# YIVEK/aom-av1-lavish

Hardware: AMD Instinct MI355X
Metric: superblocks/s (fwd_txfm+quant+SAD RDO inner loop), 1080p cpu-used=6, 1/2/4/8 GPU (higher is better)
Workload: dtype int32; 1 GPU; rdo: 1920x1080 8-bit frame per step; C2 fwd_txfm2d + quantize_fp (qindex 128) of all 14 TX sizes <=32x32 x every valid TX type + C3 DIAMOND full-pel search of every 16x16 block x 7 refs (downsampled SAD, MV_COST_ENTROPY default nmv context, sadperbit 4, errorperbit 31, cost list, step_param 0; candidate rows from the references' tiled copy, rebuilt per step); 510 SB64/frame; parallelism=frame-per-rank x1, legs=C3 on a second stream beside C2 (C3 in at most 384 workgroups)

## Files before the change

### aom-av1-lavish_amd/csrc/mcomp_lj.hip

```cpp
#include <atomic>

#include "mcomp_dev.h"
#include "txq_dev.h"

namespace lavish {
namespace {

constexpr int kLjJobs = 8;
constexpr int kMvDecHalf = 2047;
constexpr int kMvDecN = 2 * kMvDecHalf + 1;

__device__ __forceinline__ uint32_t group_min8(uint32_t v) {
  v = min(v, (uint32_t)__builtin_amdgcn_update_dpp(0, (int)v, 0xB1, 0xF, 0xF, false));
  v = min(v, (uint32_t)__builtin_amdgcn_update_dpp(0, (int)v, 0x4E, 0xF, 0xF, false));
  v = min(v, (uint32_t)__builtin_amdgcn_update_dpp(0, (int)v, 0x141, 0xF, 0xF, false));
  return v;
}

struct LjSrc {
  uint32_t sk[4], fr[2][4];
};

template <bool SKIP>
__device__ __forceinline__ uint32_t lj_sad(const Ctx& c, const LjSrc& s, int l, int r, int cc) {
// ... 3 lines not shown
    uint32_t t[4];
    load_row<4>(c.tiles + tile_off(c, c.oy + r + 2 * l, x), t);
#pragma unroll
    for (int i = 0; i < 4; ++i) acc = sad4(s.sk[i], t[i], acc);
  } else {
#pragma unroll
    for (int k = 0; k < 2; ++k) {
      uint32_t t[4];
      load_row<4>(c.tiles + tile_off(c, c.oy + r + l + 8 * k, x), t);
#pragma unroll
      for (int i = 0; i < 4; ++i) acc = sad4(s.fr[k][i], t[i], acc);
    }
  }
  acc = group_sum8(acc);
  return SKIP ? 2 * acc : acc;
}

__device__ __forceinline__ int lj_var(const Ctx& c, const LjSrc& s, int l, int r, int cc) {
  int sum = 0;
  uint32_t sse = 0;
#pragma unroll
  for (int k = 0; k < 2; ++k) {
    uint32_t t[4];
    load_row<4>(c.ref + (int64_t)(r + l + 8 * k) * c.rs + cc, t);
#pragma unroll
    for (int i = 0; i < 4; ++i) var_acc(s.fr[k][i], t[i], sum, sse);
  }
  const uint32_t ts = group_sum8((uint32_t)sum), tq = group_sum8(sse);
  const uint32_t var = tq - (uint32_t)(((int64_t)(int)ts * (int)ts) / 256);
  return (int)var + mv_cost(c, r, cc);
}

template <bool SKIP, int N>
__device__ __forceinline__ void lj_sads(const Ctx& c, const LjSrc& s, int l,
                                        __amdgpu_buffer_rsrc_t trs, int oob, const int (&r)[N],
                                        const int (&cc)[N], const bool (&v)[N],
                                        uint32_t (&out)[N]) {
  constexpr int RW = SKIP ? 1 : 2;
  u32x4 t[N][RW];
#pragma unroll
  for (int i = 0; i < N; ++i)
#pragma unroll
    for (int k = 0; k < RW; ++k) {
      const int y = c.oy + r[i] + (SKIP ? 2 * l : l + 8 * k);
      t[i][k] = __builtin_amdgcn_raw_buffer_load_b128(
          trs, v[i] ? (int)tile_off(c, y, c.ox + cc[i]) : oob, 0, 0);
    }
#pragma unroll
  for (int i = 0; i < N; ++i) {
    uint32_t acc = 0;
#pragma unroll
    for (int k = 0; k < RW; ++k) {
      const uint32_t* q = SKIP ? s.sk : s.fr[k];
      acc = sad4(q[0], t[i][k].x, acc);
      acc = sad4(q[1], t[i][k].y, acc);
      acc = sad4(q[2], t[i][k].z, acc);
      acc = sad4(q[3], t[i][k].w, acc);
    }
    acc = group_sum8(acc);
    out[i] = SKIP ? 2 * acc : acc;
  }
}

__device__ __forceinline__ uint32_t scatter_sum8(const uint32_t (&p)[8], int l) {
  const bool hi = l & 4, m1 = l & 2, m0 = l & 1;
  uint32_t q[4], r[2];
#pragma unroll
  for (int k = 0; k < 4; ++k) {
    const uint32_t send = hi ? p[k] : p[k + 4];
    const uint32_t keep = hi ? p[k + 4] : p[k];
    q[k] = keep + (uint32_t)__builtin_amdgcn_update_dpp(0, (int)send, 0x141, 0xF, 0xF, false);
  }
#pragma unroll
  for (int k = 0; k < 2; ++k) {
    const uint32_t send = m1 ? q[k] : q[k + 2];
    const uint32_t keep = m1 ? q[k + 2] : q[k];
    r[k] = keep + (uint32_t)__builtin_amdgcn_update_dpp(0, (int)send, 0x4E, 0xF, 0xF, false);
  }
  const uint32_t send = m0 ? r[0] : r[1];
  const uint32_t keep = m0 ? r[1] : r[0];
  return keep + (uint32_t)__builtin_amdgcn_update_dpp(0, (int)send, 0xB1, 0xF, 0xF, false);
}

__device__ __forceinline__ uint32_t lj_step_sad(const LjSrc& s, __amdgpu_buffer_rsrc_t trs,
                                                int oob, const uint32_t (&off)[8],
                                                const bool (&v)[8], int l) {
  u32x4 t[8];
#pragma unroll
  for (int i = 0; i < 8; ++i)
    t[i] = __builtin_amdgcn_raw_buffer_load_b128(trs, v[i] ? (int)off[i] : oob, 0, 0);
  uint32_t p[8];
#pragma unroll
  for (int i = 0; i < 8; ++i) {
    uint32_t acc = sad4(s.sk[0], t[i].x, 0);
    acc = sad4(s.sk[1], t[i].y, acc);
    acc = sad4(s.sk[2], t[i].z, acc);
    p[i] = sad4(s.sk[3], t[i].w, acc);
  }
  return 2 * scatter_sum8(p, l);
}

__device__ __forceinline__ MvRate mvsad_rate_dec(const Ctx& c, const int32_t* dec, int row,
                                                 int col) {
  if (dec == nullptr) return mvsad_rate(c, row, col);
  const int kr = row - c.full_ref_row, kc = col - c.full_ref_col;
  const int joint = (kc != 0) | ((kr != 0) << 1);
  typedef const __attribute__((address_space(1))) int32_t* gi32;
  return MvRate{((gi32)c.mvjcost)[joint], ((gi32)dec)[kr + kMvDecHalf],
                ((gi32)dec)[kc + kMvDecHalf + kMvDecN]};
}

template <bool SKIP>
__device__ void lj_pass(const Ctx& c, const LjSrc& s, int l, __amdgpu_buffer_rsrc_t trs, int oob,
                        const int32_t* dec, bool run, int step_param, bool want_cl,
                        uint32_t* res, int& steps,
                        int& searches, int& br, int& bc, int& sme, int (&cl)[5]) {
  const int srow = min(max(br, c.row_min), c.row_max);
  const int scol = min(max(bc, c.col_min), c.col_max);
  const int sdr = site_dr(l), sdc = site_dc(l);
  uint32_t c0;
  {
    const int r1[1] = {srow}, c1[1] = {scol};
    const bool v1[1] = {true};
    uint32_t o1[1];
    lj_sads<SKIP, 1>(c, s, l, trs, oob, r1, c1, v1, o1);
    c0 = o1[0] + mvsad_finish(c, mvsad_rate_dec(c, dec, srow, scol), srow, scol);
  }
  const int further = kMaxSteps - 1 - step_param;
  bool active = run;
  bool first = true;
  int n = 0, row = srow, col = scol, stp = kMaxSteps - step_param - 1, center = 0, nres = 0;
  bool offc = false;
  uint32_t best = c0;
  while (__builtin_amdgcn_ballot_w64(active) != 0) {
    const int rad = 1 << stp;
    const int rl = row + sdr * rad, cl_ = col + sdc * rad;
    const bool vl = cl_ >= c.col_min && cl_ <= c.col_max && rl >= c.row_min && rl <= c.row_max;
    MvRate mr = {0, 0, 0};
    if (vl && active) mr = mvsad_rate_dec(c, dec, rl, cl_);
    uint32_t mine = 0;
    constexpr int NS = SKIP ? 8 : 4;
    if constexpr (SKIP) {
      const bool up = row - rad >= c.row_min, dn = row + rad <= c.row_max;
      const bool lf = col - rad >= c.col_min, rt = col + rad <= c.col_max;
      const int y0 = c.oy + row + 2 * l, x0 = c.ox + col;
      uint32_t off[8];
      bool vv[8];
      if (stp > 0) {
        const int yb = (y0 & 1) * c.fsz + ((y0 >> 1) << 5), d16 = rad << 4;
        const int f32 = c.fh << 5;
        auto xo = [&](int x) { return __mul24(x >> 4, f32) + (x & 15); };
        const int xm = xo(x0 - rad), xc = xo(x0), xp = xo(x0 + rad);
#pragma unroll
        for (int t = 0; t < 8; ++t) {
          const int dr = site_dr(t), dc = site_dc(t);
          off[t] = (uint32_t)((dr < 0 ? yb - d16 : dr > 0 ? yb + d16 : yb) +
                              (dc < 0 ? xm : dc > 0 ? xp : xc));
        }
      } else {
#pragma unroll
        for (int t = 0; t < 8; ++t) off[t] = tile_off(c, y0 + site_dr(t), x0 + site_dc(t));
      }
#pragma unroll
      for (int t = 0; t < 8; ++t) {
        const int dr = site_dr(t), dc = site_dc(t);
        vv[t] = active && (dr < 0 ? up : dr > 0 ? dn : true) && (dc < 0 ? lf : dc > 0 ? rt : true);
      }
      if (active) mine = lj_step_sad(s, trs, oob, off, vv, l);
    } else
    if (active)
#pragma unroll
    for (int h = 0; h < 8 / NS; ++h) {
      int rr[NS], cc[NS];
      bool vv[NS];
      uint32_t sd[NS];
#pragma unroll
      for (int i = 0; i < NS; ++i) {
        const int t = h * NS + i;
        rr[i] = row + site_dr(t) * rad;
        cc[i] = col + site_dc(t) * rad;
        vv[i] = active && cc[i] >= c.col_min && cc[i] <= c.col_max && rr[i] >= c.row_min &&
                rr[i] <= c.row_max;
      }
      lj_sads<SKIP, NS>(c, s, l, trs, oob, rr, cc, vv, sd);
#pragma unroll
      for (int i = 0; i < NS; ++i) mine = l == h * NS + i ? sd[i] : mine;
    }
    const uint32_t key =
        (((mine + mvsad_finish(c, mr, rl, cl_)) << 3) | (uint32_t)l) | (vl ? 0u : ~0u);
    const uint32_t kmin = group_min8(key);
    if (active) {
      ++steps;
      if (kmin < (best << 3)) {
        best = kmin >> 3;
        const int i = (int)(kmin & 7);
        row += site_dr(i) * rad;
        col += site_dc(i) * rad;
        offc = true;
      }
      if (!offc) ++center;
      if (--stp < 0) {
        if (l == 0) res[nres] = ((uint32_t)(uint16_t)row << 16) | (uint16_t)col;
        ++nres;
        ++searches;
        if (first) n = center;
        else if (center) n += center;
        first = false;
        if (n < further) {
          ++n;
          row = srow;
          col = scol;
          best = c0;
          stp = kMaxSteps - (step_param + n) - 1;
          center = 0;
          offc = false;
        } else {
          active = false;
          stp = 0;
        }
      }
    }
  }
  wave_sync();
  if (!run) return;
  for (int i = 0; i < nres; ++i) {
    const uint32_t p = res[i];
    const int r = (int16_t)(p >> 16), cc = (int16_t)(p & 0xFFFF);
    const int v = lj_var(c, s, l, r, cc);
    if (i == 0 || v < sme) {
      sme = v;
      br = r;
      bc = cc;
    }
  }
  if (want_cl) {
    int rr[5], cc[5];
    bool vv[5];
    uint32_t sd[5];
    MvRate m[5];
#pragma unroll
    for (int t = 0; t < 5; ++t) {
      rr[t] = br + (t == 2 ? 1 : t == 4 ? -1 : 0);
      cc[t] = bc + (t == 1 ? -1 : t == 3 ? 1 : 0);
      vv[t] = t == 0 ||
              (cc[t] >= c.col_min && cc[t] <= c.col_max && rr[t] >= c.row_min && rr[t] <= c.row_max);
      m[t] = mvsad_rate_dec(c, dec, vv[t] ? rr[t] : br, vv[t] ? cc[t] : bc);
    }
    lj_sads<SKIP, 5>(c, s, l, trs, oob, rr, cc, vv, sd);
#pragma unroll
    for (int t = 0; t < 5; ++t)
      cl[t] = vv[t] ? (int)(sd[t] + mvsad_finish(c, m[t], rr[t], cc[t])) : INT_MAX;
  }
}

__device__ __forceinline__ void lj_jobs(
    const uint8_t* __restrict__ src, int ss, const uint8_t* __restrict__ ref, int rs,
    const LavishRefTiles& tiles, const Job* __restrict__ jobs, int njobs, int step_param,
    const LavishMvCostParams& cost, const int32_t* dec, int skip,
    LavishDiamondResult* __restrict__ out, int32_t* __restrict__ cost_lists, int j0,
    uint32_t* res);

template <int WPG>
__device__ __forceinline__ void lj_group(
    const uint8_t* __restrict__ src, int ss, const uint8_t* __restrict__ ref, int rs,
    const LavishRefTiles& tiles, const Job* __restrict__ jobs, int njobs, int step_param,
    const LavishMvCostParams& cost, const int32_t* dec, int skip,
    LavishDiamondResult* __restrict__ out, int32_t* __restrict__ cost_lists, int vwg, int nvwg) {
  __shared__ uint32_t res_s[WPG][kLjJobs][kMaxSteps];
  const int wg = (vwg & 7) * (nvwg >> 3) + (vwg >> 3);
  const int lane = threadIdx.x & 63;
  const int wave = WPG == 1 ? 0 : threadIdx.x >> 6;
  const int j0 = (wg * WPG + wave) * kLjJobs;
  if (j0 >= njobs) return;
  lj_jobs(src, ss, ref, rs, tiles, jobs, njobs, step_param, cost, dec, skip, out, cost_lists, j0,
          res_s[wave][lane >> 3]);
}

__device__ __forceinline__ void lj_jobs(
    const uint8_t* __restrict__ src, int ss, const uint8_t* __restrict__ ref, int rs,
    const LavishRefTiles& tiles, const Job* __restrict__ jobs, int njobs, int step_param,
    const LavishMvCostParams& cost, const int32_t* dec, int skip,
    LavishDiamondResult* __restrict__ out, int32_t* __restrict__ cost_lists, int j0,
    uint32_t* res) {
  const int lane = threadIdx.x & 63;
  const int jg = lane >> 3, l = lane & 7;
  const int j = min(j0 + jg, njobs - 1);
  const bool mine_job = j0 + jg < njobs;
  const Job jb = jobs[j];
  Ctx c;
  c.src = src + jb.src_off;
  c.ref = ref + jb.ref_off;
  c.ss = ss;
  c.rs = rs;
  c.col_min = jb.col_min;
  c.col_max = jb.col_max;
  c.row_min = jb.row_min;
  c.row_max = jb.row_max;
  c.ref_mv_row = jb.ref_mv_row;
  c.ref_mv_col = jb.ref_mv_col;
  c.full_ref_row = rawpel(jb.ref_mv_row);
  c.full_ref_col = rawpel(jb.ref_mv_col);
  c.cost_type = cost.mv_cost_type;
  c.sad_lambda = sad_lambda(cost.mv_cost_type);
  c.sse_lambda = sse_lambda(cost.mv_cost_type);
  c.sad_per_bit = cost.sad_per_bit;
  c.error_per_bit = cost.error_per_bit;
  const bool ent = cost.mv_cost_type == 0;
  c.mvjcost = ent ? cost.mvjcost : kZeroRate;
  c.mvcost0 = ent ? cost.mvcost[0] : kZeroRate;
  c.mvcost1 = ent ? cost.mvcost[1] : kZeroRate;
  c.tiles = tiles.data;
  c.fh = tiles.field_rows;
  c.fsz = (int)tiles.field_bytes;
  c.oy = (int)(jb.ref_off / rs);
  c.ox = (int)(jb.ref_off - (int64_t)c.oy * rs);
  const int oob = (int)(2 * tiles.field_bytes);
  const __amdgpu_buffer_rsrc_t trs =
      __builtin_amdgcn_make_buffer_rsrc((void*)tiles.data, 0, oob, 0x00020000);
  LjSrc s;
  load_row<4>(c.src + (int64_t)(2 * l) * ss, s.sk);
  load_row<4>(c.src + (int64_t)l * ss, s.fr[0]);
  load_row<4>(c.src + (int64_t)(l + 8) * ss, s.fr[1]);
  const bool want_cl = cost_lists != nullptr;
  int cl[5] = {INT_MAX, INT_MAX, INT_MAX, INT_MAX, INT_MAX};
  int steps = 0, searches = 0, sme = 0;
  int br = jb.start_row, bc = jb.start_col;
  bool full = true;
  if (skip) {
    lj_pass<true>(c, s, l, trs, oob, dec, true, step_param, want_cl, res, steps, searches, br, bc,
                  sme, cl);
    uint32_t all = 0;
#pragma unroll
    for (int k = 0; k < 2; ++k) {
      uint32_t t[4];
      load_row<4>(c.ref + (int64_t)(br + l + 8 * k) * rs + bc, t);
#pragma unroll
      for (int i = 0; i < 4; ++i) all = sad4(s.fr[k][i], t[i], all);
    }
    const int sad = (int)group_sum8(all);
    const int ssad = (int)(2 * group_sum8((l & 1) ? 0u : all));
    full = sad > 16 && abs(ssad - sad) * 10 >= max(sad, 1) * 9;
    if (full) {
      br = jb.start_row;
      bc = jb.start_col;
    }
  }
  if (__builtin_amdgcn_ballot_w64(full) != 0)
    lj_pass<false>(c, s, l, trs, oob, dec, full, step_param, want_cl, res, steps, searches, br, bc,
                   sme, cl);
  if (!mine_job) return;
  if (l == 0) {
    LavishDiamondResult r;
    r.best_row = (int16_t)br;
    r.best_col = (int16_t)bc;
    r.bestsme = sme;
    r.steps = steps;
    r.searches = searches;
    out[j] = r;
  }
  if (want_cl && l < 5) {
    const int v = l == 0 ? cl[0] : l == 1 ? cl[1] : l == 2 ? cl[2] : l == 3 ? cl[3] : cl[4];
    cost_lists[5 * (int64_t)j + l] = v;
  }
}

#ifndef LAVISH_LJ_WAVES
#define LAVISH_LJ_WAVES 4
#endif
template <int WPG>
__global__ __launch_bounds__(64 * WPG, LAVISH_LJ_WAVES) void diamond_lj_kernel(
    const uint8_t* __restrict__ src, int ss, const uint8_t* __restrict__ ref, int rs,
    LavishRefTiles tiles, const Job* __restrict__ jobs, int njobs, int step_param,
    LavishMvCostParams cost, const int32_t* dec, int skip, LavishDiamondResult* __restrict__ out,
    int32_t* __restrict__ cost_lists, int nvwg) {
  for (int v = blockIdx.x; v < nvwg; v += gridDim.x)
    lj_group<WPG>(src, ss, ref, rs, tiles, jobs, njobs, step_param, cost, dec, skip, out,
                  cost_lists, v, nvwg);
}

constexpr int kLjQueueStride = 16;

template <int WPG>
__global__ __launch_bounds__(64 * WPG, LAVISH_LJ_WAVES) void diamond_lj_dyn_kernel(
    const uint8_t* __restrict__ src, int ss, const uint8_t* __restrict__ ref, int rs,
    LavishRefTiles tiles, const Job* __restrict__ jobs, int njobs, int step_param,
    LavishMvCostParams cost, const int32_t* dec, int skip, LavishDiamondResult* __restrict__ out,
    int32_t* __restrict__ cost_lists, int* __restrict__ queue) {
  __shared__ uint32_t res_s[WPG][kLjJobs][kMaxSteps];
  const int units = (njobs + kLjJobs - 1) / kLjJobs;
  const int x = blockIdx.x & 7;
  const int u0 = units * x / 8, u1 = units * (x + 1) / 8;
  const int lane = threadIdx.x & 63;
  const int wave = WPG == 1 ? 0 : threadIdx.x >> 6;
  uint32_t* res = res_s[wave][lane >> 3];
  int* q = queue + x * kLjQueueStride;
  for (;;) {
    int t = 0;
    if (lane == 0) t = __hip_atomic_fetch_add(q, 1, __ATOMIC_RELAXED, __HIP_MEMORY_SCOPE_AGENT);
    t = __builtin_amdgcn_readfirstlane(t);
    if (u0 + t >= u1) break;
    lj_jobs(src, ss, ref, rs, tiles, jobs, njobs, step_param, cost, dec, skip, out, cost_lists,
            (u0 + t) * kLjJobs, res);
  }
}

__global__ void lj_queue_zero(int* __restrict__ queue) {
  if (threadIdx.x < 8 * kLjQueueStride) queue[threadIdx.x] = 0;
}

struct LjLaunch {
  const uint8_t* src;
  int ss;
  const uint8_t* ref;
  int rs;
  LavishRefTiles tiles;
  const Job* jobs;
  int njobs, step_param;
  LavishMvCostParams cost;
  const int32_t* dec;
  int skip;
  LavishDiamondResult* out;
  int32_t* cost_lists;
  int nvwg;
  int units;
  int every;
};

__global__ __launch_bounds__(256, 4) void txq_search_kernel(TxqDispatch d, TxqArgs a0, TxqArgs a1,
                                                            TxqArgs a2, TxqArgs a3, TxqArgs a4,
                                                            TxqArgs a5, TxqArgs a6, TxqArgs a7,
                                                            TxqArgs a8, LjLaunch c) {
  __shared__ __attribute__((aligned(16))) char lds[class_lds(0)];
  const int u = blockIdx.x >> 3, x = blockIdx.x & 7;
  const int k = u / c.every;
  if (u - k * c.every == 0 && k < c.units) {
    lj_group<4>(c.src, c.ss, c.ref, c.rs, c.tiles, c.jobs, c.njobs, c.step_param, c.cost, c.dec,
                c.skip, c.out, c.cost_lists, k * 8 + x, c.nvwg);
    return;
  }
  const int before = min((u + c.every - 1) / c.every, c.units);
  txq_multi_body<0>(d, a0, a1, a2, a3, a4, a5, a6, a7, a8, (u - before) * 8 + x, lds);
}

__global__ __launch_bounds__(256) void mvcost_dec_kernel(const int32_t* __restrict__ mvcost0,
                                                         const int32_t* __restrict__ mvcost1,
                                                         int32_t* __restrict__ dec,
                                                         int* __restrict__ queue) {
  const int i = blockIdx.x * 256 + threadIdx.x;
  if (queue != nullptr && i < 8 * kLjQueueStride) queue[i] = 0;
  if (i >= 2 * kMvDecN) return;
  const int k = (i % kMvDecN) - kMvDecHalf;
  dec[i] = (i < kMvDecN ? mvcost0 : mvcost1)[8 * k];
}

thread_local StreamScratch t_mvdec;

static std::atomic<int> g_lj_cap{0};
static int lj_grid_cap() { return g_lj_cap.load(std::memory_order_relaxed); }
static std::atomic<int> g_lj_queue{1};

constexpr int kTilesK = 8, kTilesF = 32, kTilesC = kTilesK + 1;
__global__ __launch_bounds__(256) void ref_tiles_kernel(const uint8_t* __restrict__ ref,
                                                        int stride, int rows, int nstrips,
                                                        int fh, uint8_t* __restrict__ out,
                                                        int ktiles, int ftiles) {
  __shared__ u32x4 seg[kTilesF][kTilesC];
  const int t = threadIdx.x;
  int b = blockIdx.x;
  const int kt = b % ktiles;
  b /= ktiles;
  const int ft = b % ftiles;
  const int f = b / ftiles;
  const int k0 = kt * kTilesK, fy0 = ft * kTilesF;
  for (int idx = t; idx < kTilesF * kTilesC; idx += 256) {
    const int i = idx / kTilesC, m = idx - i * kTilesC;
    const int y = 2 * (fy0 + i) + f, x = 16 * (k0 + m);
    u32x4 v = {0u, 0u, 0u, 0u};
    if (y < rows && x < stride) {
      const uint8_t* p = ref + (int64_t)y * stride + x;
      if (x + 16 <= stride) {
        const u32x4u w = *(const __attribute__((address_space(1))) u32x4u*)p;
        v = u32x4{w.x, w.y, w.z, w.w};
      } else {
        uint32_t q[4] = {0u, 0u, 0u, 0u};
        for (int j = 0; j < 16 && x + j < stride; ++j) q[j >> 2] |= (uint32_t)p[j] << (8 * (j & 3));
        v = u32x4{q[0], q[1], q[2], q[3]};
      }
    }
    seg[i][m] = v;
  }
  __syncthreads();
  for (int q = t; q < kTilesK * kTilesF * 2; q += 256) {
    const int kk = q >> 6, i = (q >> 1) & (kTilesF - 1), h = q & 1;
    const int k = k0 + kk, fy = fy0 + i;
    if (k < nstrips && fy < fh)
      *(u32x4*)(out + ((((int64_t)f * nstrips + k) * fh + fy) << 5) + 16 * h) = seg[i][kk + h];
  }
}

}

void launch_lj(const uint8_t* src, int ss, const uint8_t* ref, int rs, const LavishRefTiles& t,
               const LavishDiamondJob* jobs, int njobs, int step_param,
               const LavishMvCostParams& cost, int skip, LavishDiamondResult* out,
               int32_t* cost_lists, hipStream_t s) {
  const int waves = (njobs + kLjJobs - 1) / kLjJobs;
  constexpr int wpg = 4;
  const int nwg = (((waves + wpg - 1) / wpg) + 7) & ~7;
  const int cap = lj_grid_cap();
  const int grid = cap > 0 && cap < nwg ? cap : nwg;
  const bool dyn = grid < nwg && g_lj_queue.load(std::memory_order_relaxed);
  constexpr size_t kDecBytes = 2 * kMvDecN * sizeof(int32_t);
  const size_t qbytes = dyn ? 8 * kLjQueueStride * sizeof(int) : 0;
  int32_t* dec = nullptr;
  int* queue = nullptr;
  char* scr = nullptr;
  if (cost.mv_cost_type == 0 || dyn) {
    scr = (char*)t_mvdec.acquire(kDecBytes + qbytes, s);
    if (dyn) queue = (int*)(scr + kDecBytes);
  }
  if (cost.mv_cost_type == 0) {
    dec = (int32_t*)scr;
    hipLaunchKernelGGL(mvcost_dec_kernel, dim3((2 * kMvDecN + 255) / 256), dim3(256), 0,
                       s, cost.mvcost[0], cost.mvcost[1], dec, queue);
  } else if (dyn) {
    hipLaunchKernelGGL(lj_queue_zero, dim3(1), dim3(8 * kLjQueueStride), 0, s, queue);
  }
  if (dyn)
    hipLaunchKernelGGL(diamond_lj_dyn_kernel<wpg>, dim3(grid), dim3(64 * wpg), 0, s, src,
                       ss, ref, rs, t, (const Job*)jobs, njobs, step_param, cost,
                       (const int32_t*)dec, skip, out, cost_lists, queue);
  else
    hipLaunchKernelGGL(diamond_lj_kernel<wpg>, dim3(grid), dim3(64 * wpg), 0, s, src, ss,
                       ref, rs, t, (const Job*)jobs, njobs, step_param, cost,
                       (const int32_t*)dec, skip, out, cost_lists, nwg);
  if (scr) t_mvdec.release(s);
}

}

using namespace lavish;

extern "C" int lavish_set_search_schedule(int queued) {
  if (queued != 0 && queued != 1) return -1;
  lavish::g_lj_queue.store(queued, std::memory_order_relaxed);
  return 0;
}

extern "C" int lavish_set_search_workgroup_cap(int workgroups) {
  if (workgroups < 0) return -1;
  lavish::g_lj_cap.store((workgroups + 7) & ~7, std::memory_order_relaxed);
  return 0;
}

static int64_t tiles_nstrips(int stride) { return (stride + 15) / 16; }

extern "C" int64_t lavish_ref_tiles_bytes(int stride, int rows) {
  if (stride <= 0 || rows <= 0) return -1;
  return 2 * tiles_nstrips(stride) * ((rows + 1) / 2) * 32;
}

extern "C" int lavish_ref_tiles_build(const uint8_t* ref, int stride, int rows, uint8_t* data,
                                      LavishRefTiles* tiles, void* stream) {
  const int64_t bytes = lavish_ref_tiles_bytes(stride, rows);
  if (ref == nullptr || data == nullptr || tiles == nullptr || bytes <= 0) return -1;
  if (bytes >= ((int64_t)1 << 31)) return -1;
  const int nstrips = (int)tiles_nstrips(stride), fh = (rows + 1) / 2;
  tiles->data = data;
  tiles->field_bytes = (int64_t)nstrips * fh * 32;
  tiles->field_rows = fh;
  tiles->stride = stride;
  const int ktiles = (nstrips + kTilesK - 1) / kTilesK, ftiles = (fh + kTilesF - 1) / kTilesF;
  hipLaunchKernelGGL(ref_tiles_kernel, dim3((unsigned)(2 * ktiles * ftiles)), dim3(256), 0,
                     (hipStream_t)stream, ref, stride, rows, nstrips, fh, data, ktiles, ftiles);
  LAVISH_CHECK(hipGetLastError());
  return 0;
}

extern "C" int lavish_txq_frame_search(
    const int16_t* residual, int stride, int width, int height, uint32_t size_mask,
    const uint32_t* type_masks, int bit_depth, int quant_kind, const LavishQuantParams* qp,
    int32_t* const* qcoeff, int32_t* const* dqcoeff, uint16_t* const* eob, const uint8_t* src,
    int src_stride, const uint8_t* ref, int ref_stride, const LavishRefTiles* tiles,
    const LavishDiamondJob* jobs, int njobs, int step_param, const LavishMvCostParams* cost,
    int use_downsampled_sad, LavishDiamondResult* out, int32_t* cost_lists, int every,
    void* stream) {
  const hipStream_t s = (hipStream_t)stream;
  if (every < 1) return -6;
  if (tiles == nullptr || tiles->data == nullptr || tiles->stride != ref_stride) return -5;
  if (step_param < 0 || step_param >= kMaxSteps) return -1;
  if (!mv_cost_ok(cost)) return -2;
  uint32_t cls0 = 0;
  for (int t = 0; t < 19; ++t)
    if (((size_mask >> t) & 1) && tx_w(t) <= 32 && tx_h(t) <= 32 && !txq_class(t)) cls0 |= 1u << t;
  int rc = 0;
  if (size_mask & ~cls0) {
    rc = txq_frame(residual, stride, width, height, size_mask & ~cls0, type_masks, bit_depth,
                   quant_kind, qp, qcoeff, dqcoeff, eob, s);
    if (rc) return rc;
  }
  TxqMulti m;
  int g = 0;
  rc = txq_frame_plan(residual, stride, width, height, cls0, type_masks, bit_depth, quant_kind, qp,
                      qcoeff, dqcoeff, eob, 0, m, g);
  if (rc) return rc;
  LjLaunch c{};
  c.src = src;
  c.ss = src_stride;
  c.ref = ref;
  c.rs = ref_stride;
  c.tiles = *tiles;
  c.jobs = (const Job*)jobs;
  c.njobs = njobs > 0 ? njobs : 0;
  c.step_param = step_param;
  c.cost = *cost;
  c.skip = use_downsampled_sad;
  c.out = out;
  c.cost_lists = cost_lists;
  const int waves = (c.njobs + kLjJobs - 1) / kLjJobs;
  c.nvwg = (((waves + 3) / 4) + 7) & ~7;
  c.units = c.nvwg / 8;
  if (c.units > 0 && cost->mv_cost_type == 0) {
    c.dec = (const int32_t*)t_mvdec.acquire(2 * kMvDecN * sizeof(int32_t), s);
    hipLaunchKernelGGL(mvcost_dec_kernel, dim3((2 * kMvDecN + 255) / 256), dim3(256), 0, s,
                       cost->mvcost[0], cost->mvcost[1], (int32_t*)c.dec, (int*)nullptr);
  }
  const int u2 = g / 8, ut = u2 + c.units;
// ... 9 lines not shown
```

### aom-av1-lavish_amd/lavish_dsp/motion.py

```python
import ctypes

import numpy as np

from . import _lib, _stream_ptr

JOB_DTYPE = np.dtype([("src_off", "<i8"), ("ref_off", "<i8"), ("start_row", "<i2"),
                      ("start_col", "<i2"), ("ref_mv_row", "<i2"), ("ref_mv_col", "<i2"),
                      ("col_min", "<i2"), ("col_max", "<i2"), ("row_min", "<i2"),
                      ("row_max", "<i2")], align=True)
RESULT_DTYPE = np.dtype([("best_row", "<i2"), ("best_col", "<i2"), ("bestsme", "<i4"),
                         ("steps", "<i4"), ("searches", "<i4")], align=True)
assert JOB_DTYPE.itemsize == 32 and RESULT_DTYPE.itemsize == 16

MV_COST_ENTROPY, MV_COST_L1_LOWRES, MV_COST_L1_MIDRES, MV_COST_L1_HDRES, MV_COST_NONE = range(5)
SEARCH_METHODS = {"diamond": 0, "nstep": 1, "nstep_8pt": 2, "hex": 4, "bigdia": 5, "square": 6,
                  "fast_hex": 7, "fast_diamond": 8, "fast_bigdia": 9, "vfast_diamond": 10}
MV_MAX = (1 << 14) - 1
MI_SIZE = 4
AOM_INTERP_EXTEND = 4
MAX_FULL_PEL_VAL = (1 << 10) - 1
MV_LOW, MV_UPP = -(1 << 14), 1 << 14

_vp, _i32 = ctypes.c_void_p, ctypes.c_int32
_lib.lavish_diamond_search_batch.argtypes = [_vp, _i32, _vp, _i32, _i32, _i32, _vp, _i32, _i32,
# ... 30 lines not shown
_lib.lavish_full_pixel_search_batch_tiled.restype = _i32


class MeshParams(ctypes.Structure):
    _fields_ = [("run_mesh_search", ctypes.c_int32), ("force_mesh_thresh", ctypes.c_int32),
                ("prune_mesh_search", ctypes.c_int32),
                ("mesh_search_mv_diff_threshold", ctypes.c_int32),
                ("fine_search_interval", ctypes.c_int32), ("is_intra_mode", ctypes.c_int32),
                ("range", ctypes.c_int32 * 4), ("interval", ctypes.c_int32 * 4)]

    @classmethod
    def make(cls, patterns, run_mesh_search=0, force_mesh_thresh=0x7FFFFFFF,
             prune_mesh_search=0, mesh_search_mv_diff_threshold=4, fine_search_interval=0,
             is_intra_mode=0):
        m = cls(run_mesh_search, force_mesh_thresh, prune_mesh_search,
                mesh_search_mv_diff_threshold, fine_search_interval, is_intra_mode)
        for i, (r, iv) in enumerate(patterns):
            m.range[i], m.interval[i] = r, iv
        return m


_lib.lavish_full_pixel_search_batch_mesh.argtypes = [
    _vp, _i32, _vp, _i32, ctypes.POINTER(RefTilesDesc), _i32, _i32, _vp, _i32, _i32, _i32,
    ctypes.POINTER(MvCostParams), _i32, ctypes.POINTER(MeshParams), _vp, _vp, _vp]
_lib.lavish_full_pixel_search_batch_mesh.restype = _i32
if hasattr(_lib, "lavish_set_search_workgroup_cap"):
    _lib.lavish_set_search_workgroup_cap.argtypes = [_i32]
    _lib.lavish_set_search_workgroup_cap.restype = _i32
if hasattr(_lib, "lavish_set_search_schedule"):
    _lib.lavish_set_search_schedule.argtypes = [_i32]
    _lib.lavish_set_search_schedule.restype = _i32


class RefTiles:

    def __init__(self, ref, stride=None):
        import torch
        assert ref.dtype == torch.uint8 and ref.is_contiguous()
        self.ref = ref
        self.stride = int(stride if stride is not None else ref.shape[-1])
        self.rows = ref.numel() // self.stride
        n = _lib.lavish_ref_tiles_bytes(self.stride, self.rows)
        if n <= 0:
            raise ValueError("lavish_ref_tiles_bytes rejected (%d, %d)" % (self.stride, self.rows))
        self.data = torch.empty(n, dtype=torch.uint8, device=ref.device)
        self.desc = RefTilesDesc()

    def build(self, stream=None):
        rc = _lib.lavish_ref_tiles_build(_vp(self.ref.data_ptr()), self.stride, self.rows,
                                         _vp(self.data.data_ptr()), ctypes.byref(self.desc),
                                         _stream_ptr(stream))
        if rc != 0:
            raise ValueError("lavish_ref_tiles_build rejected its arguments (rc=%d)" % rc)
        return self


class MvCosts:

    def __init__(self, mvjcost, mvcost, device="cuda"):
        import torch
        mvcost = np.ascontiguousarray(mvcost, np.int32)
        if mvcost.shape != (2, 2 * MV_MAX + 1) or np.shape(mvjcost) != (4,):
            raise ValueError("mvjcost[4] and mvcost[2][%d] expected" % (2 * MV_MAX + 1))
        self.mvjcost = torch.from_numpy(np.ascontiguousarray(mvjcost, np.int32)).to(device)
        self.mvcost = torch.from_numpy(mvcost).to(device)

    def cost_params(self, sad_per_bit, error_per_bit, mv_cost_type=MV_COST_ENTROPY):
        c = MvCostParams(mv_cost_type, sad_per_bit, error_per_bit, 0)
        c.mvjcost = self.mvjcost.data_ptr()
        row = self.mvcost.stride(0) * 4
        c.mvcost[0] = self.mvcost.data_ptr() + 4 * MV_MAX
        c.mvcost[1] = self.mvcost.data_ptr() + row + 4 * MV_MAX
        c._owner = self
        return c


def set_search_workgroup_cap(workgroups):
    rc = _lib.lavish_set_search_workgroup_cap(int(workgroups))
    if rc:
        raise ValueError("lavish_set_search_workgroup_cap(%r): %d" % (workgroups, rc))


def set_search_schedule(queued):
    rc = _lib.lavish_set_search_schedule(1 if queued else 0)
    if rc:
        raise ValueError("lavish_set_search_schedule(%r): %d" % (queued, rc))


def default_mv_cost_tables(allow_hp=False):
    import os
    d = np.load(os.path.join(os.path.dirname(os.path.abspath(__file__)), "data",
                             "nmv_cost_default.npz"))
    t = "hp" if allow_hp else "lp"
    return d["mvjcost_" + t], d["mvcost_" + t]


def sad_per_bit(qindex, bit_depth=8):
    from . import build_quant_params
    q = int(build_quant_params(bit_depth, qindex).dequant[1]) / 4.0
    if bit_depth == 10:
        q /= 4.0
    elif bit_depth == 12:
        q /= 16.0
    return int(0.0418 * q + 2.4107)


def error_per_bit(rdmult):
    return max(rdmult >> 6, 1)


def l1_cost_params(mv_cost_type=MV_COST_L1_HDRES):
    return MvCostParams(mv_cost_type, 0, 0, 0)


def block_mv_limits(mi_rows, mi_cols, mi_row, mi_col, mi_height, mi_width, border):
    e2 = 2 * AOM_INTERP_EXTEND
    row_min = max(-(mi_row * MI_SIZE + border - e2), -((mi_row + mi_height) * MI_SIZE + e2))
    row_max = min((mi_rows - mi_row - mi_height) * MI_SIZE + border - e2,
                  (mi_rows - mi_row) * MI_SIZE + e2)
    col_min = max(-(mi_col * MI_SIZE + border - e2), -((mi_col + mi_width) * MI_SIZE + e2))
    col_max = min((mi_cols - mi_col - mi_width) * MI_SIZE + border - e2,
                  (mi_cols - mi_col) * MI_SIZE + e2)
    return col_min, col_max, row_min, row_max


def subpel_limits(lim, ref_mv=(0, 0)):
    col_min, col_max, row_min, row_max = lim
    max_mv = MAX_FULL_PEL_VAL * 8
    r, c = ref_mv
    minc = max(col_min * 8, c - max_mv)
    maxc = min(col_max * 8, c + max_mv)
    minr = max(row_min * 8, r - max_mv)
    maxr = min(row_max * 8, r + max_mv)
    maxc, maxr = max(minc, maxc), max(minr, maxr)
    return (max(MV_LOW + 1, minc), min(MV_UPP - 1, maxc), max(MV_LOW + 1, minr),
            min(MV_UPP - 1, maxr))


def mv_limits(mi_rows, mi_cols, mi_row, mi_col, mi_height, mi_width, border, ref_mv=(0, 0)):
    col_min, col_max, row_min, row_max = block_mv_limits(mi_rows, mi_cols, mi_row, mi_col,
                                                         mi_height, mi_width, border)
    r, c = ref_mv
    cmin = max(((c + 7) >> 3) - MAX_FULL_PEL_VAL, (MV_LOW >> 3) + 1)
    rmin = max(((r + 7) >> 3) - MAX_FULL_PEL_VAL, (MV_LOW >> 3) + 1)
    cmax = min((c >> 3) + MAX_FULL_PEL_VAL, (MV_UPP >> 3) - 1)
    rmax = min((r >> 3) + MAX_FULL_PEL_VAL, (MV_UPP >> 3) - 1)
    col_min, row_min = max(col_min, cmin), max(row_min, rmin)
    col_max, row_max = min(col_max, cmax), min(row_max, rmax)
    return col_min, max(col_min, col_max), row_min, max(row_min, row_max)


def frame_jobs(width, height, stride, border, plane_bytes, bw, bh, nrefs, ref_mv=(0, 0),
               start_mv=(0, 0), mv_border=None):
    mi_rows = ((height + 7) & ~7) // MI_SIZE
    mi_cols = ((width + 7) & ~7) // MI_SIZE
    nbx, nby = width // bw, height // bh
    n = nbx * nby
    one = np.zeros(n, JOB_DTYPE)
    ys = np.repeat(np.arange(nby) * bh, nbx)
    xs = np.tile(np.arange(nbx) * bw, nby)
    one["src_off"] = (ys + border) * stride + xs + border
    mb = border if mv_border is None else mv_border
    lim = np.array([mv_limits(mi_rows, mi_cols, y // MI_SIZE, x // MI_SIZE, bh // MI_SIZE,
                              bw // MI_SIZE, mb, ref_mv) for y, x in zip(ys, xs)])
    one["col_min"], one["col_max"], one["row_min"], one["row_max"] = lim.T
    one["start_row"], one["start_col"] = start_mv
    one["ref_mv_row"], one["ref_mv_col"] = ref_mv
# ... 218 lines not shown
```

Measured before the change: 776,700 SB64/s.

## Add refill walk kernel that recycles 8-lane groups across diamond searches

Adds schedule mode 2, which splits the skip-mode diamond search into a persistent walk kernel and a separate finish kernel. In the walk kernel each wave keeps a small shared-memory pool of jobs and hands a new job to any 8-lane group whose walk has ended. This removes idle lanes caused by searches of uneven length. Walk results go to a scratch record per job, and the finish kernel reads them back to do variance selection and cost lists. The mode only runs when schedule 2 is selected, and it adds an extra launch plus global traffic for the records.

Measured after the change: 768,900 SB64/s. -1.0%, worse.

```diff
diff --git a/aom-av1-lavish_amd/csrc/mcomp_lj.hip b/aom-av1-lavish_amd/csrc/mcomp_lj.hip
--- a/aom-av1-lavish_amd/csrc/mcomp_lj.hip
+++ b/aom-av1-lavish_amd/csrc/mcomp_lj.hip
@@ -109,6 +109,7 @@
   return keep + (uint32_t)__builtin_amdgcn_update_dpp(0, (int)send, 0xB1, 0xF, 0xF, false);
 }
 
+template <bool ISSUE_ALL = false>
 __device__ __forceinline__ uint32_t lj_step_sad(const LjSrc& s, __amdgpu_buffer_rsrc_t trs,
                                                 int oob, const uint32_t (&off)[8],
                                                 const bool (&v)[8], int l) {
@@ -116,6 +117,7 @@
 #pragma unroll
   for (int i = 0; i < 8; ++i)
     t[i] = __builtin_amdgcn_raw_buffer_load_b128(trs, v[i] ? (int)off[i] : oob, 0, 0);
+  if constexpr (ISSUE_ALL) __builtin_amdgcn_sched_barrier(0);
   uint32_t p[8];
 #pragma unroll
   for (int i = 0; i < 8; ++i) {
@@ -137,11 +139,87 @@
                 ((gi32)dec)[kc + kMvDecHalf + kMvDecN]};
 }
 
+__device__ __forceinline__ void lj_skip_sites(const Ctx& c, int row, int col, int stp, int l,
+                                              bool active, uint32_t (&off)[8], bool (&vv)[8]) {
+  const int rad = 1 << stp;
+  const bool up = row - rad >= c.row_min, dn = row + rad <= c.row_max;
+  const bool lf = col - rad >= c.col_min, rt = col + rad <= c.col_max;
+  const int y0 = c.oy + row + 2 * l, x0 = c.ox + col;
+  if (stp > 0) {
+    const int yb = (y0 & 1) * c.fsz + ((y0 >> 1) << 5), d16 = rad << 4;
+    const int f32 = c.fh << 5;
+    auto xo = [&](int x) { return __mul24(x >> 4, f32) + (x & 15); };
+    const int xm = xo(x0 - rad), xc = xo(x0), xp = xo(x0 + rad);
+#pragma unroll
+    for (int t = 0; t < 8; ++t) {
+      const int dr = site_dr(t), dc = site_dc(t);
+      off[t] = (uint32_t)((dr < 0 ? yb - d16 : dr > 0 ? yb + d16 : yb) +
+                          (dc < 0 ? xm : dc > 0 ? xp : xc));
+    }
+  } else {
+#pragma unroll
+    for (int t = 0; t < 8; ++t) off[t] = tile_off(c, y0 + site_dr(t), x0 + site_dc(t));
+  }
+#pragma unroll
+  for (int t = 0; t < 8; ++t) {
+    const int dr = site_dr(t), dc = site_dc(t);
+    vv[t] = active && (dr < 0 ? up : dr > 0 ? dn : true) && (dc < 0 ? lf : dc > 0 ? rt : true);
+  }
+}
+
+struct LjWalk {
+  int row, col, stp, center, n, nres;
+  bool first, offc;
+  uint32_t best;
+};
+
+__device__ __forceinline__ void lj_walk_begin(LjWalk& w, int srow, int scol, uint32_t c0,
+                                              int step_param) {
+  w.row = srow;
+  w.col = scol;
+  w.best = c0;
+  w.stp = kMaxSteps - step_param - 1;
+  w.center = w.n = w.nres = 0;
+  w.first = true;
+  w.offc = false;
+}
+
+template <class Put>
+__device__ __forceinline__ bool lj_advance(LjWalk& w, uint32_t kmin, int srow, int scol,
+                                           uint32_t c0, int step_param, Put&& put) {
+  const int rad = 1 << w.stp;
+  if (kmin < (w.best << 3)) {
+    w.best = kmin >> 3;
+    const int i = (int)(kmin & 7);
+    w.row += site_dr(i) * rad;
+    w.col += site_dc(i) * rad;
+    w.offc = true;
+  }
+  if (!w.offc) ++w.center;
+  if (--w.stp >= 0) return false;
+  put(w.nres, ((uint32_t)(uint16_t)w.row << 16) | (uint16_t)w.col);
+  ++w.nres;
+  if (w.first) w.n = w.center;
+  else if (w.center) w.n += w.center;
+  w.first = false;
+  if (w.n < kMaxSteps - 1 - step_param) {
+    ++w.n;
+    w.row = srow;
+    w.col = scol;
+    w.best = c0;
+    w.stp = kMaxSteps - (step_param + w.n) - 1;
+    w.center = 0;
+    w.offc = false;
+    return false;
+  }
+  w.stp = 0;
+  return true;
+}
+
 template <bool SKIP>
-__device__ void lj_pass(const Ctx& c, const LjSrc& s, int l, __amdgpu_buffer_rsrc_t trs, int oob,
-                        const int32_t* dec, bool run, int step_param, bool want_cl,
-                        uint32_t* res, int& steps,
-                        int& searches, int& br, int& bc, int& sme, int (&cl)[5]) {
+__device__ void lj_walk(const Ctx& c, const LjSrc& s, int l, __amdgpu_buffer_rsrc_t trs, int oob,
+                        const int32_t* dec, bool run, int step_param, int br, int bc,
+                        uint32_t* res, int& nres, int& steps, int& searches) {
   const int srow = min(max(br, c.row_min), c.row_max);
   const int scol = min(max(bc, c.col_min), c.col_max);
   const int sdr = site_dr(l), sdc = site_dc(l);
@@ -153,46 +231,21 @@
     lj_sads<SKIP, 1>(c, s, l, trs, oob, r1, c1, v1, o1);
     c0 = o1[0] + mvsad_finish(c, mvsad_rate_dec(c, dec, srow, scol), srow, scol);
   }
-  const int further = kMaxSteps - 1 - step_param;
   bool active = run;
-  bool first = true;
-  int n = 0, row = srow, col = scol, stp = kMaxSteps - step_param - 1, center = 0, nres = 0;
-  bool offc = false;
-  uint32_t best = c0;
+  LjWalk w;
+  lj_walk_begin(w, srow, scol, c0, step_param);
   while (__builtin_amdgcn_ballot_w64(active) != 0) {
-    const int rad = 1 << stp;
-    const int rl = row + sdr * rad, cl_ = col + sdc * rad;
+    const int rad = 1 << w.stp;
+    const int rl = w.row + sdr * rad, cl_ = w.col + sdc * rad;
     const bool vl = cl_ >= c.col_min && cl_ <= c.col_max && rl >= c.row_min && rl <= c.row_max;
     MvRate mr = {0, 0, 0};
     if (vl && active) mr = mvsad_rate_dec(c, dec, rl, cl_);
     uint32_t mine = 0;
     constexpr int NS = SKIP ? 8 : 4;
     if constexpr (SKIP) {
-      const bool up = row - rad >= c.row_min, dn = row + rad <= c.row_max;
-      const bool lf = col - rad >= c.col_min, rt = col + rad <= c.col_max;
-      const int y0 = c.oy + row + 2 * l, x0 = c.ox + col;
       uint32_t off[8];
       bool vv[8];
-      if (stp > 0) {
-        const int yb = (y0 & 1) * c.fsz + ((y0 >> 1) << 5), d16 = rad << 4;
-        const int f32 = c.fh << 5;
-        auto xo = [&](int x) { return __mul24(x >> 4, f32) + (x & 15); };
-        const int xm = xo(x0 - rad), xc = xo(x0), xp = xo(x0 + rad);
-#pragma unroll
-        for (int t = 0; t < 8; ++t) {
-          const int dr = site_dr(t), dc = site_dc(t);
-          off[t] = (uint32_t)((dr < 0 ? yb - d16 : dr > 0 ? yb + d16 : yb) +
-                              (dc < 0 ? xm : dc > 0 ? xp : xc));
-        }
-      } else {
-#pragma unroll
-        for (int t = 0; t < 8; ++t) off[t] = tile_off(c, y0 + site_dr(t), x0 + site_dc(t));
-      }
-#pragma unroll
-      for (int t = 0; t < 8; ++t) {
-        const int dr = site_dr(t), dc = site_dc(t);
-        vv[t] = active && (dr < 0 ? up : dr > 0 ? dn : true) && (dc < 0 ? lf : dc > 0 ? rt : true);
-      }
+      lj_skip_sites(c, w.row, w.col, w.stp, l, active, off, vv);
       if (active) mine = lj_step_sad(s, trs, oob, off, vv, l);
     } else
     if (active)
@@ -204,8 +257,8 @@
 #pragma unroll
       for (int i = 0; i < NS; ++i) {
         const int t = h * NS + i;
-        rr[i] = row + site_dr(t) * rad;
-        cc[i] = col + site_dc(t) * rad;
+        rr[i] = w.row + site_dr(t) * rad;
+        cc[i] = w.col + site_dc(t) * rad;
         vv[i] = active && cc[i] >= c.col_min && cc[i] <= c.col_max && rr[i] >= c.row_min &&
                 rr[i] <= c.row_max;
       }
@@ -218,38 +271,21 @@
     const uint32_t kmin = group_min8(key);
     if (active) {
       ++steps;
-      if (kmin < (best << 3)) {
-        best = kmin >> 3;
-        const int i = (int)(kmin & 7);
-        row += site_dr(i) * rad;
-        col += site_dc(i) * rad;
-        offc = true;
-      }
-      if (!offc) ++center;
-      if (--stp < 0) {
-        if (l == 0) res[nres] = ((uint32_t)(uint16_t)row << 16) | (uint16_t)col;
-        ++nres;
-        ++searches;
-        if (first) n = center;
-        else if (center) n += center;
-        first = false;
-        if (n < further) {
-          ++n;
-          row = srow;
-          col = scol;
-          best = c0;
-          stp = kMaxSteps - (step_param + n) - 1;
-          center = 0;
-          offc = false;
-        } else {
-          active = false;
-          stp = 0;
-        }
-      }
-    }
-  }
+      if (lj_advance(w, kmin, srow, scol, c0, step_param, [&](int i, uint32_t p) {
+            if (l == 0) res[i] = p;
+            ++searches;
+          }))
+        active = false;
+    }
+  }
+  nres = w.nres;
   wave_sync();
-  if (!run) return;
+}
+
+template <bool SKIP>
+__device__ void lj_finish(const Ctx& c, const LjSrc& s, int l, __amdgpu_buffer_rsrc_t trs,
+                          int oob, const int32_t* dec, bool want_cl, const uint32_t* res,
+                          int nres, int& br, int& bc, int& sme, int (&cl)[5]) {
   for (int i = 0; i < nres; ++i) {
     const uint32_t p = res[i];
     const int r = (int16_t)(p >> 16), cc = (int16_t)(p & 0xFFFF);
@@ -280,35 +316,51 @@
   }
 }
 
+template <bool SKIP>
+__device__ void lj_pass(const Ctx& c, const LjSrc& s, int l, __amdgpu_buffer_rsrc_t trs, int oob,
+                        const int32_t* dec, bool run, int step_param, bool want_cl,
+                        uint32_t* res, int& steps,
+                        int& searches, int& br, int& bc, int& sme, int (&cl)[5]) {
+  int nres = 0;
+  lj_walk<SKIP>(c, s, l, trs, oob, dec, run, step_param, br, bc, res, nres, steps, searches);
+  if (!run) return;
+  lj_finish<SKIP>(c, s, l, trs, oob, dec, want_cl, res, nres, br, bc, sme, cl);
+}
+
+constexpr int kLjRecWords = 16, kLjRecRes = 4;
+
+template <bool WALKED = false>
 __device__ __forceinline__ void lj_jobs(
     const uint8_t* __restrict__ src, int ss, const uint8_t* __restrict__ ref, int rs,
     const LavishRefTiles& tiles, const Job* __restrict__ jobs, int njobs, int step_param,
     const LavishMvCostParams& cost, const int32_t* dec, int skip,
     LavishDiamondResult* __restrict__ out, int32_t* __restrict__ cost_lists, int j0,
-    uint32_t* res);
-
-template <int WPG>
+    uint32_t* res, const uint32_t* __restrict__ walk = nullptr);
+
+template <int WPG, bool WALKED = false>
 __device__ __forceinline__ void lj_group(
     const uint8_t* __restrict__ src, int ss, const uint8_t* __restrict__ ref, int rs,
     const LavishRefTiles& tiles, const Job* __restrict__ jobs, int njobs, int step_param,
     const LavishMvCostParams& cost, const int32_t* dec, int skip,
-    LavishDiamondResult* __restrict__ out, int32_t* __restrict__ cost_lists, int vwg, int nvwg) {
+    LavishDiamondResult* __restrict__ out, int32_t* __restrict__ cost_lists, int vwg, int nvwg,
+    const uint32_t* __restrict__ walk = nullptr) {
   __shared__ uint32_t res_s[WPG][kLjJobs][kMaxSteps];
   const int wg = (vwg & 7) * (nvwg >> 3) + (vwg >> 3);
   const int lane = threadIdx.x & 63;
   const int wave = WPG == 1 ? 0 : threadIdx.x >> 6;
   const int j0 = (wg * WPG + wave) * kLjJobs;
   if (j0 >= njobs) return;
-  lj_jobs(src, ss, ref, rs, tiles, jobs, njobs, step_param, cost, dec, skip, out, cost_lists, j0,
-          res_s[wave][lane >> 3]);
-}
-
+  lj_jobs<WALKED>(src, ss, ref, rs, tiles, jobs, njobs, step_param, cost, dec, skip, out,
+                  cost_lists, j0, res_s[wave][lane >> 3], walk);
+}
+
+template <bool WALKED>
 __device__ __forceinline__ void lj_jobs(
     const uint8_t* __restrict__ src, int ss, const uint8_t* __restrict__ ref, int rs,
     const LavishRefTiles& tiles, const Job* __restrict__ jobs, int njobs, int step_param,
     const LavishMvCostParams& cost, const int32_t* dec, int skip,
     LavishDiamondResult* __restrict__ out, int32_t* __restrict__ cost_lists, int j0,
-    uint32_t* res) {
+    uint32_t* res, const uint32_t* __restrict__ walk) {
   const int lane = threadIdx.x & 63;
   const int jg = lane >> 3, l = lane & 7;
   const int j = min(j0 + jg, njobs - 1);
@@ -354,8 +406,20 @@
   int br = jb.start_row, bc = jb.start_col;
   bool full = true;
   if (skip) {
-    lj_pass<true>(c, s, l, trs, oob, dec, true, step_param, want_cl, res, steps, searches, br, bc,
-                  sme, cl);
+    if constexpr (WALKED) {
+      typedef const __attribute__((address_space(1))) uint32_t* gu32;
+      const gu32 rec = (gu32)(walk + (int64_t)j * kLjRecWords);
+      const int nres = (int)rec[0];
+      steps = (int)rec[1];
+      searches = (int)rec[2];
+      if (l < nres) res[l] = rec[kLjRecRes + l];
+      if (l + 8 < nres) res[l + 8] = rec[kLjRecRes + 8 + l];
+      wave_sync();
+      lj_finish<true>(c, s, l, trs, oob, dec, want_cl, res, nres, br, bc, sme, cl);
+    } else {
+      lj_pass<true>(c, s, l, trs, oob, dec, true, step_param, want_cl, res, steps, searches, br,
+                    bc, sme, cl);
+    }
     uint32_t all = 0;
 #pragma unroll
     for (int k = 0; k < 2; ++k) {
@@ -433,6 +497,193 @@
 
 __global__ void lj_queue_zero(int* __restrict__ queue) {
   if (threadIdx.x < 8 * kLjQueueStride) queue[threadIdx.x] = 0;
+}
+
+constexpr int kLjPool = 16;
+constexpr int kLjPoolLow = 4;
+
+struct LjPoolRec {
+  Job jb;
+  int oy, ox, j, pad;
+};
+
+template <int WPG>
+__global__ __launch_bounds__(64 * WPG, LAVISH_LJ_WAVES) void diamond_lj_walk_kernel(
+    const uint8_t* __restrict__ src, int ss, int rs, LavishRefTiles tiles,
+    const Job* __restrict__ jobs, int njobs, int step_param, LavishMvCostParams cost,
+    const int32_t* dec, uint32_t* __restrict__ walk, int* __restrict__ queue) {
+  __shared__ LjPoolRec pool_s[WPG][kLjPool];
+  const int units = (njobs + kLjJobs - 1) / kLjJobs;
+  const int x = blockIdx.x & 7;
+  const int u0 = units * x / 8, u1 = units * (x + 1) / 8;
+  const int lane = threadIdx.x & 63;
+  const int wave = WPG == 1 ? 0 : threadIdx.x >> 6;
+  const int l = lane & 7;
+  const int sdr = site_dr(l), sdc = site_dc(l);
+  int* q = queue + x * kLjQueueStride;
+  Ctx c = {};
+  c.ss = ss;
+  c.rs = rs;
+  c.cost_type = cost.mv_cost_type;
+  c.sad_lambda = sad_lambda(cost.mv_cost_type);
+  c.sse_lambda = sse_lambda(cost.mv_cost_type);
+  c.sad_per_bit = cost.sad_per_bit;
+  c.error_per_bit = cost.error_per_bit;
+  const bool ent = cost.mv_cost_type == 0;
+  c.mvjcost = ent ? cost.mvjcost : kZeroRate;
+  c.mvcost0 = ent ? cost.mvcost[0] : kZeroRate;
+  c.mvcost1 = ent ? cost.mvcost[1] : kZeroRate;
+  c.tiles = tiles.data;
+  c.fh = tiles.field_rows;
+  c.fsz = (int)tiles.field_bytes;
+  const int oob = (int)(2 * tiles.field_bytes);
+  const __amdgpu_buffer_rsrc_t trs =
+      __builtin_amdgcn_make_buffer_rsrc((void*)tiles.data, 0, oob, 0x00020000);
+  int head = 0, cnt = 0, stage = 0, rec_n = 0, rec_j0 = 0, tq = 0;
+  bool dry = false;
+  u32x2 rj[4] = {};
+  LjSrc s = {};
+  LjWalk w = {};
+  bool walking = false;
+  int srow = 0, scol = 0, jid = 0, steps = 0;
+  uint32_t c0 = 0;
+  for (;;) {
+    head = __builtin_amdgcn_readfirstlane(head);
+    cnt = __builtin_amdgcn_readfirstlane(cnt);
+    stage = __builtin_amdgcn_readfirstlane(stage);
+    rec_n = __builtin_amdgcn_readfirstlane(rec_n);
+    rec_j0 = __builtin_amdgcn_readfirstlane(rec_j0);
+    dry = __builtin_amdgcn_readfirstlane((int)dry) != 0;
+    if (stage == 2) {
+      if (lane < rec_n) {
+        LjPoolRec r;
+        __builtin_memcpy(&r.jb, rj, sizeof(Job));
+        r.oy = (int)(r.jb.ref_off / rs);
+        r.ox = (int)(r.jb.ref_off - (int64_t)r.oy * rs);
+        r.j = rec_j0 + lane;
+        r.pad = 0;
+        pool_s[wave][(head + cnt + lane) & (kLjPool - 1)] = r;
+      }
+      cnt += rec_n;
+      stage = 0;
+    } else if (stage == 1) {
+      const int t = __builtin_amdgcn_readfirstlane(tq);
+      if (u0 + t < u1) {
+        rec_j0 = (u0 + t) * kLjJobs;
+        rec_n = min(kLjJobs, njobs - rec_j0);
+        if (lane < rec_n) {
+          typedef const __attribute__((address_space(1))) u32x2* gptr2;
+          const gptr2 p = (gptr2)(jobs + rec_j0 + lane);
+#pragma unroll
+          for (int i = 0; i < 4; ++i) rj[i] = p[i];
+        }
+        stage = 2;
+      } else {
+        dry = true;
+        stage = 0;
+      }
+    }
+    if (stage == 0 && !dry && cnt < kLjPoolLow) {
+      if (lane == 0) {
+        int z = lane;
+        asm volatile("" : "+v"(z));
+        tq = __hip_atomic_fetch_add(q + z, 1, __ATOMIC_RELAXED, __HIP_MEMORY_SCOPE_AGENT);
+      }
+      stage = 1;
+    }
+    const uint64_t im = __builtin_amdgcn_ballot_w64(!walking);
+    const int rank = (int)(__builtin_amdgcn_mbcnt_hi((uint32_t)(im >> 32),
+                                                     __builtin_amdgcn_mbcnt_lo((uint32_t)im, 0u)) >> 3);
+    const bool take = !walking && rank < cnt;
+    const int ntake = min((int)__popcll(im) >> 3, cnt);
+    if (ntake == 0 && im == ~(uint64_t)0) {
+      if (dry && stage == 0) break;
+      continue;
+    }
+    u32x4 nsk = {0u, 0u, 0u, 0u}, ts = {0u, 0u, 0u, 0u};
+    if (ntake != 0) {
+      wave_sync();
+      if (take) {
+        const LjPoolRec r = pool_s[wave][(head + rank) & (kLjPool - 1)];
+        c.col_min = r.jb.col_min;
+        c.col_max = r.jb.col_max;
+        c.row_min = r.jb.row_min;
+        c.row_max = r.jb.row_max;
+        c.full_ref_row = rawpel(r.jb.ref_mv_row);
+        c.full_ref_col = rawpel(r.jb.ref_mv_col);
+        c.oy = r.oy;
+        c.ox = r.ox;
+        jid = r.j;
+        srow = min(max((int)r.jb.start_row, c.row_min), c.row_max);
+        scol = min(max((int)r.jb.start_col, c.col_min), c.col_max);
+        {
+          typedef const __attribute__((address_space(1))) u32x4u* gptr4;
+          const u32x4u v = *(gptr4)(src + r.jb.src_off + (int64_t)(2 * l) * ss);
+          nsk = u32x4{v.x, v.y, v.z, v.w};
+        }
+        ts = __builtin_amdgcn_raw_buffer_load_b128(
+            trs, (int)tile_off(c, c.oy + srow + 2 * l, c.ox + scol), 0, 0);
+      }
+      wave_sync();
+      head = (head + ntake) & (kLjPool - 1);
+      cnt -= ntake;
+    }
+    const int rad = 1 << w.stp;
+    const int rl = take ? srow : w.row + sdr * rad, cl_ = take ? scol : w.col + sdc * rad;
+    const bool vl = cl_ >= c.col_min && cl_ <= c.col_max && rl >= c.row_min && rl <= c.row_max;
+    MvRate mr = {0, 0, 0};
+    if (vl && (walking || take)) mr = mvsad_rate_dec(c, dec, rl, cl_);
+    uint32_t mine = 0;
+    {
+      uint32_t off[8];
+      bool vv[8];
+      lj_skip_sites(c, w.row, w.col, w.stp, l, walking, off, vv);
+      if (walking) mine = lj_step_sad<true>(s, trs, oob, off, vv, l);
+    }
+    const uint32_t mvc = mvsad_finish(c, mr, rl, cl_);
+    const uint32_t key = (((mine + mvc) << 3) | (uint32_t)l) | (vl ? 0u : ~0u);
+    const uint32_t kmin = group_min8(key);
+    uint32_t sacc = sad4(nsk.x, ts.x, 0);
+    sacc = sad4(nsk.y, ts.y, sacc);
+    sacc = sad4(nsk.z, ts.z, sacc);
+    sacc = sad4(nsk.w, ts.w, sacc);
+    asm volatile("" : "+v"(sacc));
+    if (walking) {
+      ++steps;
+      typedef __attribute__((address_space(1))) uint32_t* gu32;
+      const gu32 rec = (gu32)(walk + (int64_t)jid * kLjRecWords);
+      if (lj_advance(w, kmin, srow, scol, c0, step_param, [&](int i, uint32_t p) {
+            if (l == 0) rec[kLjRecRes + i] = p;
+          })) {
+        walking = false;
+        if (l == 0) {
+          rec[0] = (uint32_t)w.nres;
+          rec[1] = (uint32_t)steps;
+          rec[2] = (uint32_t)w.nres;
+        }
+      }
+    }
+    if (take) {
+      c0 = 2 * group_sum8(sacc) + mvc;
+      s.sk[0] = nsk.x;
+      s.sk[1] = nsk.y;
+      s.sk[2] = nsk.z;
+      s.sk[3] = nsk.w;
+      lj_walk_begin(w, srow, scol, c0, step_param);
+      steps = 0;
+      walking = true;
+    }
+  }
+}
+
+template <int WPG>
+__global__ __launch_bounds__(64 * WPG, LAVISH_LJ_WAVES) void diamond_lj_finish_kernel(
+    const uint8_t* __restrict__ src, int ss, const uint8_t* __restrict__ ref, int rs,
+    LavishRefTiles tiles, const Job* __restrict__ jobs, int njobs, int step_param,
+    LavishMvCostParams cost, const int32_t* dec, LavishDiamondResult* __restrict__ out,
+    int32_t* __restrict__ cost_lists, int nvwg, const uint32_t* __restrict__ walk) {
+  lj_group<WPG, true>(src, ss, ref, rs, tiles, jobs, njobs, step_param, cost, dec, 1, out,
+                      cost_lists, blockIdx.x, nvwg, walk);
 }
 
 struct LjLaunch {
@@ -536,15 +787,20 @@
   const int nwg = (((waves + wpg - 1) / wpg) + 7) & ~7;
   const int cap = lj_grid_cap();
   const int grid = cap > 0 && cap < nwg ? cap : nwg;
-  const bool dyn = grid < nwg && g_lj_queue.load(std::memory_order_relaxed);
-  constexpr size_t kDecBytes = 2 * kMvDecN * sizeof(int32_t);
+  const int sched = g_lj_queue.load(std::memory_order_relaxed);
+  const bool dyn = grid < nwg && sched != 0;
+  const bool refill = dyn && sched == 2 && skip != 0;
+  constexpr size_t kDecBytes = (2 * kMvDecN * sizeof(int32_t) + 63) & ~(size_t)63;
   const size_t qbytes = dyn ? 8 * kLjQueueStride * sizeof(int) : 0;
+  const size_t wbytes = refill ? (size_t)njobs * kLjRecWords * sizeof(uint32_t) : 0;
   int32_t* dec = nullptr;
   int* queue = nullptr;
+  uint32_t* walk = nullptr;
   char* scr = nullptr;
   if (cost.mv_cost_type == 0 || dyn) {
-    scr = (char*)t_mvdec.acquire(kDecBytes + qbytes, s);
+    scr = (char*)t_mvdec.acquire(kDecBytes + qbytes + wbytes, s);
     if (dyn) queue = (int*)(scr + kDecBytes);
+    if (refill) walk = (uint32_t*)(scr + kDecBytes + qbytes);
   }
   if (cost.mv_cost_type == 0) {
     dec = (int32_t*)scr;
@@ -553,7 +809,14 @@
   } else if (dyn) {
     hipLaunchKernelGGL(lj_queue_zero, dim3(1), dim3(8 * kLjQueueStride), 0, s, queue);
   }
-  if (dyn)
+  if (refill) {
+    hipLaunchKernelGGL(diamond_lj_walk_kernel<wpg>, dim3(grid), dim3(64 * wpg), 0, s, src, ss,
+                       rs, t, (const Job*)jobs, njobs, step_param, cost, (const int32_t*)dec,
+                       walk, queue);
+    hipLaunchKernelGGL(diamond_lj_finish_kernel<wpg>, dim3(nwg), dim3(64 * wpg), 0, s, src, ss,
+                       ref, rs, t, (const Job*)jobs, njobs, step_param, cost,
+                       (const int32_t*)dec, out, cost_lists, nwg, (const uint32_t*)walk);
+  } else if (dyn)
     hipLaunchKernelGGL(diamond_lj_dyn_kernel<wpg>, dim3(grid), dim3(64 * wpg), 0, s, src,
                        ss, ref, rs, t, (const Job*)jobs, njobs, step_param, cost,
                        (const int32_t*)dec, skip, out, cost_lists, queue);
@@ -569,7 +832,7 @@
 using namespace lavish;
 
 extern "C" int lavish_set_search_schedule(int queued) {
-  if (queued != 0 && queued != 1) return -1;
+  if (queued < 0 || queued > 2) return -1;
   lavish::g_lj_queue.store(queued, std::memory_order_relaxed);
   return 0;
 }
diff --git a/aom-av1-lavish_amd/lavish_dsp/motion.py b/aom-av1-lavish_amd/lavish_dsp/motion.py
--- a/aom-av1-lavish_amd/lavish_dsp/motion.py
+++ b/aom-av1-lavish_amd/lavish_dsp/motion.py
@@ -136,7 +136,7 @@
 
 
 def set_search_schedule(queued):
-    rc = _lib.lavish_set_search_schedule(1 if queued else 0)
+    rc = _lib.lavish_set_search_schedule(int(queued))
     if rc:
         raise ValueError("lavish_set_search_schedule(%r): %d" % (queued, rc))
 
```
